# joe5saia/Hmc.jl

Hardware: AMD Instinct MI355X
Metric: Gibbs draws/sec (whole node), 3-state T=1000 x256 windows per GPU (higher is better)
Workload: dtype f64

## Files before the change

hmc.jl_amd/csrc/gibbs_device.hpp:

```cpp
#pragma once
#include <hip/hip_runtime.h>
#include <stdint.h>

#include "../../include/hmcg.h"
#include "round5.hpp"

namespace hmcg {

enum { SITE_SIG2 = 0, SITE_MU = 1, SITE_RHO = 2, SITE_A = 3, SITE_X = 4, SITE_NOISE = 5 };
constexpr int GAMMA_MAX_ATTEMPTS = 64;
constexpr double INVSQRT2PI = 0.3989422804014327;
constexpr double TWO_PI = 6.283185307179586476925286766559;
constexpr double EPS64 = 2.220446049250313e-16;

struct KernelParams {
    const double* Y;
    const int32_t* T;
    const double* yreal;
    int32_t ldY, W, H;
    int32_t sweep_begin;
    int32_t sweep_end;
    int32_t resume;
    int32_t final_launch;
    int32_t horizons[HMCG_MAXH];
// ... 456 lines not shown
__device__ __forceinline__ uint32_t map_const(int v)
{
    uint32_t m = 0;
#pragma unroll
    for (int s = 0; s < K; ++s) m |= (uint32_t)v << (4 * s);
    return m;
}
__device__ __forceinline__ int map_apply(uint32_t m, int s) { return (int)((m >> (4 * s)) & 15u); }

constexpr uint32_t BMAP_IDENTITY = 0x03020100u;
__device__ __forceinline__ uint32_t bmap_const(int v) { return (uint32_t)v * 0x01010101u; }
__device__ __forceinline__ uint32_t bmap_compose(uint32_t a, uint32_t b) { return __builtin_amdgcn_perm(a, a, b); }
__device__ __forceinline__ int bmap_apply(uint32_t m, int s) { return (int)((m >> (8 * s)) & 0xFFu); }
constexpr int DPP_ROW_SHL1 = 0x101, DPP_ROW_SHL2 = 0x102, DPP_ROW_SHL4 = 0x104, DPP_ROW_SHL8 = 0x108, DPP_WAVE_SHL1 = 0x130;

template <int K>
__device__ inline void matmul_small(double (&out)[K][K], const double (&a)[K][K], const double (&b)[K][K])
{
    double t[K][K];
#pragma unroll
    for (int i = 0; i < K; ++i)
#pragma unroll
        for (int j = 0; j < K; ++j) {
            double acc = 0.0;
#pragma unroll
            for (int k = 0; k < K; ++k) acc += a[i][k] * b[k][j];
            t[i][j] = acc;
        }
#pragma unroll
    for (int i = 0; i < K; ++i)
#pragma unroll
        for (int j = 0; j < K; ++j) out[i][j] = t[i][j];
}

template <int K>
__device__ inline double forecast_value(const double (&mu)[K], const double (&A)[K][K], const double (&pe)[K], int h)
{
    double M[K][K], v[K];
#pragma unroll
    for (int i = 0; i < K; ++i) {
        v[i] = mu[i];
#pragma unroll
        for (int j = 0; j < K; ++j) M[i][j] = A[i][j];
    }
    for (unsigned hh = (unsigned)h; hh != 0; hh >>= 1) {
        if (hh & 1u) {
            double nv[K];
#pragma unroll
            for (int i = 0; i < K; ++i) {
                double acc = 0.0;
#pragma unroll
                for (int j = 0; j < K; ++j) acc = fma(M[i][j], v[j], acc);
                nv[i] = acc;
            }
#pragma unroll
            for (int i = 0; i < K; ++i) v[i] = nv[i];
        }
        if (hh > 1u) matmul_small<K>(M, M, M);
    }
    double f = 0.0;
#pragma unroll
    for (int i = 0; i < K; ++i) f = fma(pe[i], v[i], f);
    return f;
}


template <int K>
struct ThetaBuf {
    double mu[K], sig2[K], isd[K], coef[K], rho[K];
    double A[K][K];
    double pi_end[K];
};

template <int K>
struct RngBuf {
    static constexpr int NG = K + K * K;
    double x[NG][2];
    double lu[NG][2];
    double uu[NG][2];
    double z[K];
    double rho[K];
};

template <int K, int L, int NT, bool SIG>
struct SweepShared {
    static constexpr int NW = NT / 64;
    static constexpr int NCNT = K + K * K;
    static constexpr int NF = K * K + (SIG ? K : 0);
    static constexpr int FW = (64 * L < 1024) ? 10 : 16;
    static constexpr int FPK = 32 / FW;
    static constexpr int NPK = (NF + FPK - 1) / FPK;
    unsigned red_pk[NW][NPK];
    double red_s1[SIG ? NW : 1][K];
    double red_s2[SIG ? NW : 1][K];
    int x_end;
    double red_d1[NW][K];
    double red_d2[NW][K];
    double pivot[K];
    ThetaBuf<K> th[2];
    RngBuf<K> rb[2];
    double wtot[NW][K * K];
    double pfirst[NT + 1][K];
    uint32_t wmap[NW];
    double ulast;
    int xfirst[NT + 1];
    double bred[NW];
    int selcnt[2][8][3];
    double ux[NT * L];
    double exptab[EXPTAB_N * EXPTAB_C];
    struct OutConst { double* base; double yr; int packed; int h; };
    OutConst oc[2][64];
    double ftail[2][SIG ? HMCG_MAXTAIL : 1][K];
    double pf_rep[2][K];
    double y_last[2];
};

template <int NW>
__device__ __forceinline__ double block_sum(double v, double* bred, int wave, int lane)
{
    v = wave_sum(v);
    __syncthreads();
    if (lane == 0 && wave < NW) bred[wave] = v;
    __syncthreads();
    double t = 0.0;
#pragma unroll
    for (int w = 0; w < NW; ++w) t += bred[w];
    return t;
}
template <int NW>
__device__ __forceinline__ double block_minmax(double v, double* bred, int wave, int lane, bool is_max)
{
    v = is_max ? wave_max(v) : wave_min(v);
    __syncthreads();
    if (lane == 0 && wave < NW) bred[wave] = v;
    __syncthreads();
    double t = bred[0];
#pragma unroll
    for (int w = 1; w < NW; ++w) t = is_max ? fmax(t, bred[w]) : fmin(t, bred[w]);
    return t;
}

__device__ __forceinline__ unsigned long long order_key(double v)
{
    const long long b = __double_as_longlong(v + 0.0);
    return (unsigned long long)(b ^ ((b >> 63) | (long long)0x8000000000000000ull));
}
__device__ __forceinline__ double key_value(unsigned long long k)
{
    return __longlong_as_double((long long)((k >> 63) ? (k ^ 0x8000000000000000ull) : ~k));
}
template <int NW, int NE, typename ElemFn>
__device__ __forceinline__ unsigned long long block_select(int n, ElemFn elem, int r, int (*cnt)[8][3], int wave, int lane)
{
    unsigned long long prefix = 0ull, mask = 0ull;
    const bool mine = __builtin_amdgcn_readfirstlane(wave) < NW;
    for (int b = 62; b >= 0; b -= 2) {
        const int par = (b >> 1) & 1;
        if (mine) {
            int c0 = 0, c1 = 0, c2 = 0;
            auto one = [&](int i) __attribute__((always_inline)) {
                unsigned long long key;
                const bool live = elem(i, key);
                const bool cand = live && ((key ^ prefix) & mask) == 0ull;
                const unsigned digit = (unsigned)(key >> b) & 3u;
                c0 += __builtin_popcountll(__builtin_amdgcn_ballot_w64(cand && digit == 0u));
                c1 += __builtin_popcountll(__builtin_amdgcn_ballot_w64(cand && digit == 1u));
                c2 += __builtin_popcountll(__builtin_amdgcn_ballot_w64(cand && digit == 2u));
            };
            if constexpr (NE > 0) {
#pragma unroll
                for (int i = 0; i < NE; ++i) one(i);
            } else {
                for (int i = 0; i < n; ++i) one(i);
            }
            if (lane == 0) { cnt[par][wave][0] = c0; cnt[par][wave][1] = c1; cnt[par][wave][2] = c2; }
        }
        __syncthreads();
        int t0 = 0, t1 = 0, t2 = 0;
#pragma unroll
        for (int w = 0; w < NW; ++w) { t0 += cnt[par][w][0]; t1 += cnt[par][w][1]; t2 += cnt[par][w][2]; }
        t0 = __builtin_amdgcn_readfirstlane(t0); t1 = __builtin_amdgcn_readfirstlane(t1); t2 = __builtin_amdgcn_readfirstlane(t2);
        unsigned long long digit = 0ull;
        if (r >= t0) { r -= t0; digit = 1ull;
            if (r >= t1) { r -= t1; digit = 2ull;
                if (r >= t2) { r -= t2; digit = 3ull; } } }
        prefix |= digit << b;
        mask |= 3ull << b;
    }
    return prefix;
}

template <int K>
__device__ __forceinline__ void sort_order(const double (&mu)[K], int (&order)[K])
{
    int pos[K];
#pragma unroll
    for (int i = 0; i < K; ++i) {
        int c = 0;
#pragma unroll
        for (int j = 0; j < K; ++j) c += (mu[j] < mu[i] || (mu[j] == mu[i] && j < i)) ? 1 : 0;
        pos[i] = c;
    }
#pragma unroll
    for (int q = 0; q < K; ++q) {
        int o = 0;
#pragma unroll
        for (int i = 0; i < K; ++i) o += (pos[i] == q) ? i : 0;
        order[q] = o;
    }
}

#ifdef HMCG_STAMPS
#define HMCG_NSTAMP 20
#define HMCG_NSTAMP_ALL (HMCG_NSTAMP + 2)
#define STAMP(i)                                                          \
    do {                                                                  \
        __builtin_amdgcn_sched_barrier(0);                                \
        asm volatile("; HMCG_STAMP_MARK %0" :: "n"(i));                    \
        const unsigned long long t_ = __builtin_amdgcn_s_memtime();       \
        __builtin_amdgcn_s_waitcnt(0xC07F);                               \
        __builtin_amdgcn_sched_barrier(0);                                \
        stamp_acc[i] += t_ - stamp_prev;                                  \
        stamp_prev = t_;                                                  \
    } while (0)
#else
#define STAMP(i)
#endif


template <int K, int L, int NT, bool SIG = false, bool SMOOTH = false, int NH = 0, int OCC = 1>
__global__ __launch_bounds__(NT + 64 * NH) __attribute__((amdgpu_waves_per_eu(OCC)))
void gibbs_sweeps_kernel(const KernelParams p)
{
    static_assert(NH == 0 || (NH == 4 && NT == 256), "helper waves: 256 + 256 threads");
    static_assert(K >= 2 && K <= 4, "small-K kernel: byte-per-entry state maps (v_perm_b32 composition)");
    static_assert(NT % 64 == 0 && NT >= 128, "at least two whole waves (wave 0 draws, the others work in its shadow)");
    constexpr int NW = NT / 64;
    constexpr int KK = K * K;
    constexpr int NG = K + KK;
    static_assert(NG <= 64, "draw roles must fit wave 0");
    using Sh = SweepShared<K, L, NT, SIG>;
    __shared__ Sh sh;

    int w_ = blockIdx.x;
    int t_lo_ = INT32_MIN, t_hi_ = INT32_MAX;
    if (p.order) {
        const int n_live = p.order[0];
        t_lo_ = p.order[1]; t_hi_ = p.order[2];
        if (n_live >= 0) {
            if (w_ >= n_live) __builtin_amdgcn_endpgm();
            w_ = p.order[4 + w_];
        }
    }
    const int w = w_;
    const int tid = threadIdx.x, lane = tid & 63, wave = __builtin_amdgcn_readfirstlane(tid >> 6);
    const int T = p.T[w];
    const int t0 = tid * L;
    const int owner = (T - 1) / L, l_last = (T - 1) % L;
    const bool helper = NH > 0 && __builtin_amdgcn_readfirstlane(wave) >= NW;
    int st = 0;

    if (T < t_lo_ || T > t_hi_) __builtin_amdgcn_endpgm();
    if (T < 2 || T > NT * L || T > p.ldY) {
        if (tid == 0) flag_skipped(p, w, HMCG_ST_BAD_T);
        return;
    }

    exptab_fill(sh.exptab, tid, NT + 64 * NH);
    constexpr int XPAD = K < 4 ? K : 0;
    constexpr bool PADMARK = K < 4;
    double y[L];
    int x[L];
    bool bad = false;
#pragma unroll
    for (int l = 0; l < L; ++l) {
        const bool v = (t0 + l) < T;
        y[l] = v ? p.Y[(size_t)w * p.ldY + t0 + l] : 0.0;
        bad |= v && !isfinite(y[l]);
        x[l] = XPAD;
    }
    if (__syncthreads_or(bad ? 1 : 0)) {
        if (tid == 0) flag_skipped(p, w, HMCG_ST_NONFINITE);
        return;
    }
    int sb = T, se = T;
    double yreal[SIG ? L : 1];
    const double kfac = SIG ? 1.0 / (1.0 + p.kappa) : 1.0;
    if constexpr (SIG) {
        if (p.sig_range) { sb = p.sig_range[2 * w]; se = p.sig_range[2 * w + 1]; }
        bool bad_range = sb < 0 || se > T || (sb < se && se != T);
        if (p.save_range) {
            const int svb = p.save_range[2 * w], sve = p.save_range[2 * w + 1];
            bad_range |= svb < 0 || sve > T || (svb < sve && p.sigvals && sve - svb > p.nsave_ld);
        }
        if (bad_range) {
            if (tid == 0) flag_skipped(p, w, HMCG_ST_BAD_RANGE);
            return;
        }
        if (sb >= se) { sb = T; se = T; }
#pragma unroll
        for (int l = 0; l < L; ++l) yreal[l] = y[l];
    }
    int tail = 0;
    if constexpr (SIG) {
        if (p.end_pos) tail = (T - 1) - p.end_pos[w];
        if (tail < 0 || tail > HMCG_MAXTAIL || tail > T - 1) {
            if (tid == 0) flag_skipped(p, w, HMCG_ST_BAD_T);
            return;
        }
    }
    (void)kfac; (void)yreal; (void)sb; (void)se; (void)tail;

    double part = 0.0;
#pragma unroll
    for (int l = 0; l < L; ++l) part += y[l];
    const double xi = block_sum<NW>(part, sh.bred, wave, lane) / (double)T;

    double pivot[K];
#pragma unroll
    for (int k = 0; k < K; ++k) pivot[k] = xi;

    const int NCK = 3 * K + K * K + 2 * p.H + K;
    if (p.resume) {
#pragma unroll
        for (int l = 0; l < L; ++l) if (t0 + l < T) x[l] = min((int)p.xstate[(size_t)w * p.ldY + t0 + l], K - 1);
        if (p.sumacc) {
#pragma unroll
            for (int k = 0; k < K; ++k) pivot[k] = p.sumacc[(size_t)w * NCK + (NCK - K) + k];
        }
    } else if (p.x_init) {
#pragma unroll
        for (int l = 0; l < L; ++l) if (t0 + l < T) x[l] = min(max(p.x_init[(size_t)w * p.ldY + t0 + l], 0), K - 1);
    } else {
        double lmin = 1.0e308, lmax = -1.0e308;
#pragma unroll
        for (int l = 0; l < L; ++l) if (t0 + l < T) { lmin = fmin(lmin, y[l]); lmax = fmax(lmax, y[l]); }
        const double ymin = block_minmax<NW>(lmin, sh.bred, wave, lane, false);
        const double ymax = block_minmax<NW>(lmax, sh.bred, wave, lane, true);
        unsigned long long key[L];
#pragma unroll
        for (int l = 0; l < L; ++l) key[l] = order_key(y[l]);
        const int rlo = (T - 1) / 2;
        const double med_lo = key_value(block_select<NW, L>(L, [&](int l, unsigned long long& k) __attribute__((always_inline)) { k = key[l]; return t0 + l < T; },
                                                            rlo, sh.selcnt, wave, lane));
        double med_hi = med_lo;
        if (!(T & 1)) {
            double nle = 0.0, above = 1.0e308;
#pragma unroll
            for (int l = 0; l < L; ++l) {
                if (!helper && t0 + l < T) {
                    if (y[l] <= med_lo) nle += 1.0;
                    else above = fmin(above, y[l]);
                }
            }
            const double cle = block_sum<NW>(nle, sh.bred, wave, lane);
            const double nxt = block_minmax<NW>(above, sh.bred, wave, lane, false);
            med_hi = (cle > (double)(rlo + 1)) ? med_lo : nxt;
        }
        {
#pragma clang fp contract(off)
// ... 311 lines not shown
            unsigned v = 0;
#pragma unroll
            for (int q = 0; q < Sh::FPK; ++q) {
                const int e = Sh::FPK * d + q;
                if (e < NF) v |= ((acc[e / FPW] >> (PB * (e % FPW))) & ((1u << PB) - 1u)) << (Sh::FW * q);
            }
            pk[d] = v;
        }
        wave_sum_words_lane63<NPK>(pk);
        double d1[K], d2[K], s1[SIG ? K : 1], s2[SIG ? K : 1];
#pragma unroll
        for (int i = 0; i < K; ++i) { d1[i] = 0.0; d2[i] = 0.0; }
        if constexpr (SIG) {
#pragma unroll
            for (int i = 0; i < K; ++i) { s1[i] = 0.0; s2[i] = 0.0; }
        }
#pragma unroll
        for (int l = 0; l < L; ++l) {
            double pvt = pivot[0];
#pragma unroll
            for (int k = 1; k < K; ++k) pvt = (x[l] == k) ? pivot[k] : pvt;
            const double dl = y[l] - pvt;
            const int t = t0 + l;
            const bool issig = SIG && t >= sb && t < se;
            const int xs = PADMARK ? (issig ? -1 : x[l]) : ((t < T && !issig) ? x[l] : -1);
#pragma unroll
            for (int i = 0; i < K; ++i) {
                const double dm = (xs == i) ? dl : 0.0;
                d1[i] += dm;
                d2[i] = fma(dm, dm, d2[i]);
            }
            if constexpr (SIG) {
                const int xg = issig ? x[l] : -1;
#pragma unroll
                for (int i = 0; i < K; ++i) {
                    const double dm = (xg == i) ? dl : 0.0;
                    s1[i] += dm;
                    s2[i] = fma(dm, dm, s2[i]);
                }
            }
        }
        if constexpr (SIG) {
            static_assert(!SIG || K <= 4, "signal path: transposed reduce carries 2 x 4 slots");
            double v8[8], o0, o1;
#pragma unroll
            for (int i = 0; i < 4; ++i) { v8[i] = i < K ? s1[i < K ? i : 0] : 0.0; v8[4 + i] = i < K ? s2[i < K ? i : 0] : 0.0; }
            wave_sum8_transposed(v8, lane, o0, o1);
            if ((lane & 0x3C) == 12) {
                const int i0 = lane & 2, i1 = i0 + 1;
                double* dst = (lane & 1) ? &sh.red_s2[wave][0] : &sh.red_s1[wave][0];
                if (i0 < K) dst[i0] = o0;
                if (i1 < K) dst[i1] = o1;
            }
        }
        if constexpr (K <= 4) {
            double v8[8], o0, o1;
#pragma unroll
            for (int i = 0; i < 4; ++i) { v8[i] = i < K ? d1[i] : 0.0; v8[4 + i] = i < K ? d2[i] : 0.0; }
            wave_sum8_transposed(v8, lane, o0, o1);
            if ((lane & 0x3C) == 12) {
                const int i0 = lane & 2, i1 = i0 + 1;
                double* dst = (lane & 1) ? &sh.red_d2[wave][0] : &sh.red_d1[wave][0];
                if (i0 < K) dst[i0] = o0;
                if (i1 < K) dst[i1] = o1;
            }
        } else {
#pragma unroll
            for (int i = 0; i < K; ++i) { d1[i] = wave_sum(d1[i]); d2[i] = wave_sum(d2[i]); }
            if (lane == 0) {
#pragma unroll
                for (int i = 0; i < K; ++i) { sh.red_d1[wave][i] = d1[i]; sh.red_d2[wave][i] = d2[i]; }
            }
        }
        if (lane == 63) {
#pragma unroll
            for (int d = 0; d < NPK; ++d) sh.red_pk[wave][d] = pk[d];
        }
        if (tid == 0) {
#pragma unroll
            for (int k = 0; k < K; ++k) sh.pivot[k] = pivot[k];
            sh.x_end = x_end;
        }
    };
    auto regen_y = [&](int smp, bool report) __attribute__((always_inline)) {
        if constexpr (SIG) {
            const double ssig = p.sigma_signal ? p.sigma_signal[w] : 0.0;
            const bool noisy = ssig != 0.0 || p.n_samples > 1;
            int svb = 0, sve = 0;
            if (p.save_range) { svb = p.save_range[2 * w]; sve = p.save_range[2 * w + 1]; }
            Rng gn = rng;
            gn.sweep = (uint32_t)smp;
#pragma unroll
            for (int l = 0; l < L; ++l) {
                const int t = t0 + l;
                if (noisy && t >= sb && t < se) {
                    uint32_t r[4];
                    gn.block(SITE_NOISE, 0, (uint32_t)t, r);
                    y[l] = yreal[l] + box_muller(r) * ssig;
                }
                if (report && p.sigvals && t >= svb && t < sve && t < T && (t - svb) < p.nsave_ld)
                    p.sigvals[((size_t)w * p.n_samples + smp) * p.nsave_ld + (t - svb)] = y[l];
                if (t == T - 1) sh.y_last[smp & 1] = y[l];
            }
        }
    };
    if constexpr (SIG) {
        if (p.sweep_begin % p.per_sample != 0) regen_y(p.sweep_begin / p.per_sample, false);
    }
    if (!helper) publish_stats();

    if (p.sweep_begin < p.sweep_end && shadow_wave == 0) job_prep(p.sweep_begin);

    uint32_t trips = 0;
    if constexpr (NH > 0) {
        const int ntrip = (((T + 1) >> 1) + 127) >> 7;
        constexpr int trip_wave[10] = {1, 2, 3, NW, 1, 2, 3, NW + 3, NW + 2, NW + 1};
        for (int k = 0; k < ntrip && k < 32; ++k) {
            const int wv = k < 10 ? trip_wave[k] : 1 + (k - 10) % 3;
            trips |= (wv == wave) ? (1u << k) : 0u;
        }
        trips = __builtin_amdgcn_readfirstlane(trips);
    }
    auto job_uniform_trips = [&](int sw) __attribute__((always_inline)) {
        const int nblk = (T + 1) >> 1;
        for (uint32_t m = trips; m != 0; m &= m - 1) {
            const int k = __builtin_ctz(m);
            job_uniforms(sw, k << 7, min((k << 7) + 128, nblk));
        }
    };

    double pf[L][K];
    double sm_acc[SMOOTH ? L : 1][K];
    double fm_acc[SMOOTH ? L : 1][K];
    if constexpr (SMOOTH) {
#pragma unroll
        for (int l = 0; l < L; ++l)
#pragma unroll
            for (int q = 0; q < K; ++q)
            {
                sm_acc[l][q] = (p.resume && p.pi_smooth_mean && t0 + l < T) ? p.pi_smooth_mean[((size_t)w * p.ldY + t0 + l) * K + q] : 0.0;
                fm_acc[l][q] = (p.resume && p.pi_filter_mean && t0 + l < T) ? p.pi_filter_mean[((size_t)w * p.ldY + t0 + l) * K + q] : 0.0;
            }
    }
    (void)sm_acc; (void)fm_acc;
#ifdef HMCG_STAMPS
    for (int i = 0; i < HMCG_NSTAMP; ++i) stamp_acc[i] = 0;
    stamp_prev = __builtin_amdgcn_s_memtime();
    const unsigned long long stamp_t0 = stamp_prev, stamp_r0 = __builtin_amdgcn_s_memrealtime();
#endif

    if constexpr (NH > 0) {
        if (helper) {
            for (int sweep = p.sweep_begin; sweep < p.sweep_end; ++sweep) {
                __syncthreads();
                STAMP(0);
                if (wave == PREP_WAVE && sweep + 1 < p.sweep_end) job_prep(sweep + 1);
                STAMP(15);
                job_uniform_trips(sweep);
                STAMP(1);
                __syncthreads();
                STAMP(2);
                if (sweep > p.sweep_begin) job_outputs(sweep - 1);
                STAMP(14);
                __syncthreads();
                __syncthreads();
                __syncthreads();
                STAMP(11);
            }
        }
    }

    for (int sweep = helper ? p.sweep_end : p.sweep_begin; sweep < p.sweep_end; ++sweep) {
        rng.sweep = (uint32_t)sweep;
        const int par = sweep & 1;
        ThetaBuf<K>& th = sh.th[par];
        if constexpr (SIG) {
            const int smp = sweep / p.per_sample;
            if (sweep == smp * p.per_sample) { regen_y(smp, true); publish_stats(); }
        }
        __syncthreads();
        STAMP(0);
        if (wave == 0) {
            const RngBuf<K>& rb = sh.rb[par];
            const int qi = (lane - 4) >> 2, qj = (lane - 4) & 3;
            const bool is_sig = lane < K, is_A = lane >= 4 && qi < K && qj < K;
            const bool is_g = is_sig || is_A;
            const int role = is_sig ? lane : (is_A ? K + qi * K + qj : NG);
            double shape = 1.0, bpar = 1.0, Neff = 0.0, Ssum = 0.0, rnn = 0.0;
            int cT = 0;
            {
                const int e = is_A ? (PADCNT ? qj * K + qi : role - K) : 0;
#pragma unroll
                for (int ww = 0; ww < NW; ++ww) cT += (int)((sh.red_pk[ww][e / Sh::FPK] >> (Sh::FW * (e % Sh::FPK))) & ((1u << Sh::FW) - 1u));
                cT = is_A ? cT : 0;
            }
            int rowsum = 0;
            {
                int qs = cT + __builtin_amdgcn_mov_dpp(cT, 0xB1, 0xF, 0xF, false);
                qs += __builtin_amdgcn_mov_dpp(qs, 0x4E, 0xF, 0xF, false);
#pragma unroll
                for (int i = 0; i < K; ++i) {
                    const int ri = __builtin_amdgcn_readlane(qs, 4 + 4 * i);
                    rowsum = (lane == i) ? ri : rowsum;
                }
            }
            STAMP(16);
            if (is_g) {
                const int c = is_sig ? rowsum + ((sh.x_end == role) ? 1 : 0) : cT;
                if (is_sig) {
                    double d1 = 0.0, d2 = 0.0;
#pragma unroll
                    for (int ww = 0; ww < NW; ++ww) { d1 += sh.red_d1[ww][role]; d2 += sh.red_d2[ww][role]; }
                    const double piv = sh.pivot[role];
                    const double beta = (sweep == 0) ? 1.0 : 2.0;
                    if constexpr (!SIG) {
                        Neff = (double)c;
                        const double rn = c > 0 ? rcp_fast(Neff) : 0.0;
                        const double ybar = c > 0 ? piv + d1 * rn : 0.0;
                        const double S2 = c > 0 ? fmax(d2 - d1 * d1 * rn, 0.0) : 0.0;
                        Ssum = piv * Neff + d1;
                        const double dm = ybar - xi;
                        shape = p.alpha + 0.5 * Neff;
                        rnn = rcp_fast(Neff + p.nu);
                        bpar = beta + 0.5 * S2 + 0.5 * Neff * p.nu * rnn * (dm * dm);
                    } else {
                        int Mi = 0;
                        {
                            const int e = KK + role;
#pragma unroll
                            for (int ww = 0; ww < NW; ++ww) Mi += (int)((sh.red_pk[ww][e / Sh::FPK] >> (Sh::FW * (e % Sh::FPK))) & ((1u << Sh::FW) - 1u));
                        }
                        const int Ni = c - Mi;
                        double g1 = 0.0, g2 = 0.0;
#pragma unroll
                        for (int ww = 0; ww < NW; ++ww) { g1 += sh.red_s1[ww][role]; g2 += sh.red_s2[ww][role]; }
                        const double dNi = (double)Ni, dMi = (double)Mi;
                        const double S = piv * dNi + d1, Sm = piv * dMi + g1;
                        const double S2 = Ni > 0 ? fmax(d2 - d1 * d1 / dNi, 0.0) : 0.0;
                        const double Sm2 = Mi > 0 ? fmax(g2 - g1 * g1 / dMi, 0.0) : 0.0;
                        const double totalbar = (Ni + Mi) > 0 ? (S + Sm) / (dNi + dMi) : 0.0;
                        Neff = dNi + dMi * kfac;
                        Ssum = S + Sm;
                        const double dm = totalbar - xi;
                        shape = p.alpha + 0.5 * dNi + 0.5 * dMi;
                        rnn = rcp_fast(Neff + p.nu);
                        bpar = beta + 0.5 * S2 + (0.5 * kfac) * Sm2 + 0.5 * Neff * p.nu * rnn * (dm * dm);
                    }
                } else {
                    shape = (double)(c + 1);
                }
// ... 455 lines not shown
        STAMP(8);
        int xlast = 0;
        {
            const double ulast = sh.ulast;
            double cp = 0.0;
#pragma unroll
            for (int q = 0; q < K - 1; ++q) {
                double pq = 0.0;
#pragma unroll
                for (int s = 0; s < K; ++s) pq = (order[q] == s) ? th.pi_end[s] : pq;
                cp += pq;
                xlast += (cp <= ulast) ? 1 : 0;
            }
        }
        double pfn_last[K];
#pragma unroll
        for (int s = 0; s < K; ++s) pfn_last[s] = sh.pfirst[(tid + 1 < NT) ? tid + 1 : tid][s];
        uint32_t gmap[L];
        uint32_t G = BMAP_IDENTITY;
#pragma unroll
        for (int l = L - 1; l >= 0; --l) {
            const int t = t0 + l;
            uint32_t m = 0;
            int idx_uni = 0;
            {
                double ucum = 0.0;
#pragma unroll
                for (int r = 0; r < K - 1; ++r) { ucum += 1.0 / K; idx_uni += (ucum <= ux[l]) ? 1 : 0; }
            }
#pragma unroll
            for (int s = 0; s < K; ++s) {
                const double guard = (l + 1 < L) ? pf[(l + 1 < L) ? l + 1 : l][s] : pfn_last[s];
                double tot = 0.0;
                int idx = 0;
                double cum[K];
#pragma unroll
                for (int r = 0; r < K; ++r) { tot = fma(pf[l][r], A[r][s], tot); cum[r] = tot; }
                const double thr = ux[l] * tot;
#pragma unroll
                for (int r = 0; r < K - 1; ++r) idx += (cum[r] <= thr) ? 1 : 0;
                idx = (guard > EPS64) ? idx : idx_uni;
                m |= (uint32_t)idx << (8 * s);
            }
            if constexpr (K < 4) m |= BMAP_IDENTITY & (0xFFFFFFFFu << (8 * K));
            m = (t == T - 1) ? bmap_const(xlast) : (t > T - 1 ? (PADMARK ? bmap_const(XPAD) : BMAP_IDENTITY) : m);
            gmap[l] = m;
            G = bmap_compose(m, G);
        }
        STAMP(9);
        uint32_t Hm = G;
        Hm = bmap_compose(Hm, (uint32_t)dpp_i32<DPP_ROW_SHL1, 0xF>((int)BMAP_IDENTITY, (int)Hm));
        Hm = bmap_compose(Hm, (uint32_t)dpp_i32<DPP_ROW_SHL2, 0xF>((int)BMAP_IDENTITY, (int)Hm));
        Hm = bmap_compose(Hm, (uint32_t)dpp_i32<DPP_ROW_SHL4, 0xF>((int)BMAP_IDENTITY, (int)Hm));
        Hm = bmap_compose(Hm, (uint32_t)dpp_i32<DPP_ROW_SHL8, 0xF>((int)BMAP_IDENTITY, (int)Hm));
        {
            const uint32_t R1 = (uint32_t)__builtin_amdgcn_readlane((int)Hm, 16);
            const uint32_t R2 = (uint32_t)__builtin_amdgcn_readlane((int)Hm, 32);
            const uint32_t R3 = (uint32_t)__builtin_amdgcn_readlane((int)Hm, 48);
            const uint32_t S1 = bmap_compose(R2, R3), S0 = bmap_compose(R1, S1);
            const int row = lane >> 4;
            const uint32_t after = row == 0 ? S0 : (row == 1 ? S1 : (row == 2 ? R3 : BMAP_IDENTITY));
            Hm = bmap_compose(Hm, after);
        }
        if (lane == 0) sh.wmap[wave] = Hm;
        STAMP(10);
        __syncthreads();
        STAMP(11);
        uint32_t Rw = BMAP_IDENTITY;
#pragma unroll
        for (int ww = NW - 1; ww >= 1; --ww) if (ww > wave_u) Rw = bmap_compose(sh.wmap[ww], Rw);
        const uint32_t Hx = (uint32_t)dpp_i32<DPP_WAVE_SHL1, 0xF>((int)BMAP_IDENTITY, (int)Hm);
        const uint32_t Sfx = bmap_compose(Hx, Rw);
        int sin = bmap_apply(Sfx, XPAD);
        xnext = sin;
        x_end = xlast;
#pragma unroll
        for (int l = L - 1; l >= 0; --l) {
            sin = bmap_apply(gmap[l], sin);
            x[l] = sin;
        }
#pragma unroll
        for (int k = 0; k < K; ++k) pivot[k] = mu[k];
        STAMP(12);
        publish_stats();
        STAMP(13);
    }
#ifdef HMCG_STAMPS
    if (lane == 0 && p.dbg) {
        unsigned long long* o = p.dbg + ((size_t)w * (NW + NH) + wave) * HMCG_NSTAMP_ALL;
        for (int i = 0; i < HMCG_NSTAMP; ++i) o[i] = stamp_acc[i];
        o[HMCG_NSTAMP] = __builtin_amdgcn_s_memtime() - stamp_t0;
        o[HMCG_NSTAMP + 1] = __builtin_amdgcn_s_memrealtime() - stamp_r0;
    }
#endif

    __syncthreads();
    if (p.sweep_end > p.sweep_begin) job_outputs(p.sweep_end - 1);
    if (p.xstate) {
#pragma unroll
        for (int l = 0; l < L; ++l) if (t0 + l < T) p.xstate[(size_t)w * p.ldY + t0 + l] = (uint8_t)x[l];
    }
    if (p.x_final) {
#pragma unroll
        for (int l = 0; l < L; ++l) if (t0 + l < T) p.x_final[(size_t)w * p.ldY + t0 + l] = x[l];
    }
    if (p.pif_final && p.sweep_end > p.sweep_begin) {
#pragma unroll
        for (int l = 0; l < L; ++l)
            if (t0 + l < T)
#pragma unroll
                for (int s = 0; s < K; ++s) p.pif_final[((size_t)w * p.ldY + t0 + l) * K + s] = pf[l][s];
    }
    if constexpr (SMOOTH) {
        if (p.pi_filter_mean) {
            const double sc = (p.final_launch && p.nd > 0) ? 1.0 / (double)p.nd : 1.0;
#pragma unroll
            for (int l = 0; l < L; ++l)
                if (t0 + l < T)
#pragma unroll
                    for (int q = 0; q < K; ++q) p.pi_filter_mean[((size_t)w * p.ldY + t0 + l) * K + q] = fm_acc[l][q] * sc;
        }
        if (p.pi_smooth_mean) {
            const double sc = (p.final_launch && p.nd > 0) ? 1.0 / (double)p.nd : 1.0;
#pragma unroll
            for (int l = 0; l < L; ++l)
                if (t0 + l < T)
#pragma unroll
                    for (int q = 0; q < K; ++q) p.pi_smooth_mean[((size_t)w * p.ldY + t0 + l) * K + q] = sm_acc[l][q] * sc;
        }
    }
    {
        const int orole = role_of(lane);
        if (orole >= 0) {
            if (p.sumacc) p.sumacc[(size_t)w * NCK + orole] = sum_acc;
            if (p.summary && p.final_launch)
                p.summary[(size_t)w * NS + orole] = p.nd > 0 ? sum_acc / (double)p.nd : __builtin_nan("");
            if constexpr (SIG) {
                if (p.sample_summary) {
                    const int smp = p.sweep_end / p.per_sample, kb = p.sweep_end - smp * p.per_sample - p.burnin_s;
                    if (kb > 0 && kb < p.nrun_s && smp < p.n_samples) p.sample_summary[((size_t)w * p.n_samples + smp) * NS + orole] = smp_acc;
                }
            }
        }
    }
    if (p.sumacc) {
#pragma unroll
        for (int k = 0; k < K; ++k) if (tid == k) p.sumacc[(size_t)w * NCK + (NCK - K) + k] = pivot[k];
    }
    if (st) atomicOr(&p.status[w], st);
}

}
```

hmc.jl_amd/csrc/hmcg.hip:

```cpp
#include <hip/hip_runtime.h>

#include <algorithm>
#include <chrono>
#include <cstdarg>
#include <cstdlib>
#include <cstdio>
#include <cstring>
#include <functional>
#include <mutex>
#include <string>
#include <thread>
#include <vector>

#include "gibbs_device.hpp"
#include "host_util.hpp"
#include "moments.hpp"
#include "plan.hpp"

namespace {

thread_local char g_err[512] = "";

void set_err(const char* fmt, ...)
{
// ... 249 lines not shown
{
    const size_t stride = (size_t)W + ORD_HDR;
    int32_t* meta = ord + (size_t)MAXBUCKET * stride;
    const int w = (int)(blockIdx.x * blockDim.x + threadIdx.x);
    if (w < W) {
        auto bucket_of = [&](int t) { int k = 0; for (int b = 0; b < r.nb; ++b) if (t >= r.lo[b] && t <= r.hi[b]) k = b; return k; };
        const int mine = bucket_of(T[w]);
        int32_t* list = ord + (size_t)mine * stride;
        const int pos = atomicAdd(&list[0], 1);
        list[ORD_HDR + pos] = w;
        if (w > 0 && bucket_of(T[w - 1]) != mine) atomicAdd(&meta[0], 1);
    }
    __threadfence();
    __syncthreads();
    if (threadIdx.x == 0 && atomicAdd(&meta[1], 1) == (int)gridDim.x - 1) {
        __threadfence();
        int runs = 0;
        for (int b = 0; b < r.nb; ++b) runs += atomicAdd(&ord[(size_t)b * stride], 0) > 0 ? 1 : 0;
        const bool sorted = atomicAdd(&meta[0], 0) == runs - 1 || !r.compact;
        for (int b = 0; b < r.nb; ++b) {
            int32_t* list = ord + (size_t)b * stride;
            if (sorted) list[0] = -1;
            list[1] = r.lo[b]; list[2] = r.hi[b];
        }
    }
}
size_t bucket_list_bytes(int W) { return sizeof(int32_t) * ((size_t)MAXBUCKET * ((size_t)W + ORD_HDR) + 2); }
int build_bucket_lists(const Plan& pl, const int32_t* dT, int W, int32_t* ord, hipStream_t stream)
{
    BucketRanges r{};
    r.nb = pl.nb;
    r.compact = diag_env("HMCG_NO_BUCKET_LISTS") ? 0 : 1;
    for (int b = 0; b < pl.nb; ++b) { r.lo[b] = pl.b[b].t_lo; r.hi[b] = pl.b[b].t_hi; }
    HIP_TRY(hipMemsetAsync(ord, 0, bucket_list_bytes(W), stream));
    hipLaunchKernelGGL(bucket_lists_kernel, dim3((unsigned)((W + 255) / 256)), dim3(256), 0, stream, dT, W, r, ord);
    HIP_TRY(hipGetLastError());
    return 0;
}

int launch_kernel(DeviceCtx& c, const Plan& pl, const hmcg::KernelParams& p, hipStream_t stream, const int32_t* ord)
{
    if (pl.nb > 1) {
        HIP_TRY(hipEventRecord(c.ev_fork, stream));
        for (int b = 0; b < pl.nb; ++b) {
            hipStream_t bs = b == 0 ? stream : c.bstream[b - 1];
            if (b > 0) HIP_TRY(hipStreamWaitEvent(bs, c.ev_fork, 0));
            hmcg::KernelParams q = p;
            q.order = ord + (size_t)b * ((size_t)p.W + ORD_HDR);
            const Variant* v = pl.b[b].v;
            hipLaunchKernelGGL(v->fn, dim3((unsigned)p.W), dim3((unsigned)(v->NT + 64 * v->NH)), 0, bs, q);
            HIP_TRY(hipGetLastError());
            if (b > 0) HIP_TRY(hipEventRecord(c.ev_join[b - 1], bs));
        }
        for (int b = 1; b < pl.nb; ++b) HIP_TRY(hipStreamWaitEvent(stream, c.ev_join[b - 1], 0));
        return 0;
    }
    if (pl.v) hipLaunchKernelGGL(pl.v->fn, dim3((unsigned)p.W), dim3((unsigned)(pl.v->NT + 64 * pl.v->NH)), 0, stream, p);
    else hipLaunchKernelGGL(pl.bv->fn, dim3((unsigned)p.W), dim3((unsigned)pl.bv->NT), pl.dyn, stream, p, pl.bigL);
    HIP_TRY(hipGetLastError());
    return 0;
}

void fill_timing(hmcg_timing* t, const Plan& pl, const DeviceCtx& c, double kernel_ms, int launches, double call_ms, int windows)
{
    if (!t) return;
    t->kernel_ms = kernel_ms;
    t->launches = launches;
    t->threads_per_window = pl.NT();
    t->steps_per_thread = pl.L();
    t->helper_waves = pl.NH();
    t->device = c.device;
    t->call_ms = call_ms;
    t->windows = windows;
    t->occupancy = pl.v ? pl.v->occ : 0;
    t->buckets = pl.nb > 1 ? pl.nb : 1;
    t->streaming = pl.stream ? 1 : 0;
    t->lds_bytes = (int32_t)(static_lds_bytes(pl.fptr(), 0) + pl.dyn);
}

#ifdef HMCG_STAMPS
int print_stamps(const hmcg::KernelParams& p, const Plan& pl, unsigned long long* ddbg, size_t ndbg, hipStream_t stream)
{
    static const char* names[HMCG_NSTAMP] = {"Ba wait", "param draws | shadow jobs", "Bb wait", "theta+ux+pdfs", "local product",
        "wave scan", "Bc wait", "prefix+replay+last", "Bd wait", "maps+compose", "map scan", "Be wait", "apply", "publish stats", "  (shadow: outputs)", "  (shadow: prep)", "  (param: counts+row sums)", "  (param: shapes)", "  (param: gamma)", "unused"};
    const int nwv = pl.NT() / 64 + pl.NH();
    std::vector<unsigned long long> h(ndbg);
    HIP_TRY(hipStreamSynchronize(stream));
    static int launches_seen = 0;
    static const int print_after = diag_env("HMCG_STAMPS_AFTER") ? atoi(diag_env("HMCG_STAMPS_AFTER")) : 0;
    if (launches_seen++ < print_after) return 0;
    HIP_TRY(hipMemcpy(h.data(), ddbg, ndbg * sizeof(unsigned long long), hipMemcpyDeviceToHost));
    const int nsw = p.sweep_end - p.sweep_begin;
    {
        std::vector<double> clk;
        double ticks = 0;
        for (int w = 0; w < p.W; ++w)
            for (int wv = 0; wv < nwv; ++wv) {
                const unsigned long long* o = &h[((size_t)w * nwv + wv) * HMCG_NSTAMP_ALL];
                if (o[HMCG_NSTAMP + 1]) { clk.push_back(100.0 * (double)o[HMCG_NSTAMP] / (double)o[HMCG_NSTAMP + 1]); ticks += (double)o[HMCG_NSTAMP]; }
            }
        std::sort(clk.begin(), clk.end());
        if (!clk.empty())
            fprintf(stderr, "[clock] launch %d: in-kernel clock MHz min %.0f median %.0f max %.0f (s_memtime / s_memrealtime x 100 MHz); "
                            "%.0f ticks per sweep (mean over waves)\n", launches_seen - 1, clk.front(), clk[clk.size() / 2], clk.back(),
                    ticks / (double)clk.size() / (nsw > 0 ? nsw : 1));
    }
    fprintf(stderr, "[stamps] K=%d L=%d NT=%d W=%d sweeps=%d: mean cycles per sweep by wave (s_memtime ticks)\n",
            pl.v ? pl.v->K : pl.bv->K, pl.L(), pl.NT(), p.W, nsw);
    fprintf(stderr, "%-24s", "phase");
    for (int wv = 0; wv < nwv; ++wv) fprintf(stderr, "   wave%-2d", wv);
    fprintf(stderr, "\n");
    std::vector<double> tot(nwv, 0.0);
    for (int i = 0; i < HMCG_NSTAMP; ++i) {
        fprintf(stderr, "%-24s", names[i]);
        for (int wv = 0; wv < nwv; ++wv) {
            double acc = 0;
            for (int w = 0; w < p.W; ++w) acc += (double)h[((size_t)w * nwv + wv) * HMCG_NSTAMP_ALL + i];
            acc /= (double)p.W * (nsw > 0 ? nsw : 1);
            tot[wv] += acc;
            fprintf(stderr, " %8.0f", acc);
        }
        fprintf(stderr, "\n");
    }
    fprintf(stderr, "%-24s", "total");
    for (int wv = 0; wv < nwv; ++wv) fprintf(stderr, " %8.0f", tot[wv]);
    fprintf(stderr, "\n");
    return 0;
}
#endif


int grow_shared(DeviceCtx& c, Arena& a, size_t bytes)
{
    if (a.cap >= bytes) return 0;
    HIP_TRY(hipEventSynchronize(c.ev_scr));
    if (a.ensure(bytes)) { set_err("workspace allocation failed (%zu B device)", bytes); return HMCG_E_NOMEM; }
    return 0;
}

int launch_device(DeviceCtx& c, const hmcg_config* cfg, const double* dY, const int32_t* dT, const double* dyreal, double* dmu,
                  double* dsig2, double* dA, double* dpi_end, double* dfcast, double* dsummary, int32_t* dstatus,
                  const hmcg_extras* ex, hipStream_t stream, hmcg_timing* timing)
{
    if (!dY || !dT || !dstatus) { set_err("Y, T and status are required"); return HMCG_E_BADARG; }
    Plan pl;
    int rc = plan_call(cfg, ex, cfg->W, c.cu_count, cfg->min_T, nullptr, &pl);
    if (rc) return rc;
    if (pl.needs_pif() && !(ex && ex->pif_final)) {
        set_err("pi_smooth_mean / pi_filter_mean for K >= 5 or windows beyond the register-resident kernels need extras.pif_final "
                "([W][ldY][K]: the running sweep's filtered probabilities pass through it)");
        return HMCG_E_BADARG;
    }
    if (ex && ex->corr && (!dmu || !dsig2 || !dA || !dpi_end || !dfcast)) {
        set_err("extras.corr on the device entry needs all five per-draw outputs");
        return HMCG_E_BADARG;
    }
    const bool resume = (cfg->flags & HMCG_FLAG_RESUME) != 0;
    hmcg::KernelParams p = base_params(cfg, cfg->W, dY, dT, dyreal, dstatus, ex, pl);
    p.sweep_begin = pl.sched.sweep_begin; p.sweep_end = pl.sched.sweep_end; p.final_launch = pl.sched.final_launch;
    p.resume = resume ? 1 : 0;
    p.mu = dmu; p.sig2 = dsig2; p.A = dA; p.pi_end = dpi_end; p.fcast = dfcast; p.summary = dsummary;
    p.nd_ld = p.nd; p.draw_off = 0;

    if (!resume) HIP_TRY(hipMemsetAsync(dstatus, 0, sizeof(int32_t) * (size_t)cfg->W, stream));
    const bool use_lists = pl.nb > 1;
    const bool uses_scratch = pl.bv != nullptr || (ex && ex->corr) || use_lists;
    if (uses_scratch) HIP_TRY(hipStreamWaitEvent(stream, c.ev_scr, 0));
// ... 454 lines not shown
```

Measured before the change: 54.11 million.

## Offload per-state residual sums to helper waves via shared state bytes

When helper waves are present (non-SIG, non-smooth), the main waves now pack their sampled state sequence into shared memory as bytes. After an extra barrier, helper waves load those states along with their own copy of y and compute the per-state first and second moment sums, while main waves compute only the transition counts. This splits the end-of-sweep statistics work across more waves so the critical path gets shorter. In exchange it adds an extra __syncthreads per sweep and uses more LDS for the state bytes.

```diff
diff --git a/hmc.jl_amd/csrc/gibbs_device.hpp b/hmc.jl_amd/csrc/gibbs_device.hpp
--- a/hmc.jl_amd/csrc/gibbs_device.hpp
+++ b/hmc.jl_amd/csrc/gibbs_device.hpp
@@ -562,8 +562,11 @@
     double rho[K];
 };
 
-template <int K, int L, int NT, bool SIG>
-struct SweepShared {
+template <int NXS> struct StateBytes { uint32_t xs[NXS]; };
+template <> struct StateBytes<0> {};
+
+template <int K, int L, int NT, bool SIG, int NXS = 0>
+struct SweepShared : StateBytes<NXS> {
     static constexpr int NW = NT / 64;
     static constexpr int NCNT = K + K * K;
     static constexpr int NF = K * K + (SIG ? K : 0);
@@ -719,7 +722,9 @@
     constexpr int KK = K * K;
     constexpr int NG = K + KK;
     static_assert(NG <= 64, "draw roles must fit wave 0");
-    using Sh = SweepShared<K, L, NT, SIG>;
+    constexpr bool HSTAT = NH > 0 && !SIG && !SMOOTH && !(K == 2 && L >= 3);
+    constexpr int XSW = (L + 3) / 4;
+    using Sh = SweepShared<K, L, NT, SIG, HSTAT ? NT * XSW : 0>;
     __shared__ Sh sh;
 
     int w_ = blockIdx.x;
@@ -738,6 +743,7 @@
     const int t0 = tid * L;
     const int owner = (T - 1) / L, l_last = (T - 1) % L;
     const bool helper = NH > 0 && __builtin_amdgcn_readfirstlane(wave) >= NW;
+    const int ts = (HSTAT && helper) ? t0 - NT * L : t0;
     int st = 0;
 
     if (T < t_lo_ || T > t_hi_) __builtin_amdgcn_endpgm();
@@ -754,8 +760,8 @@
     bool bad = false;
 #pragma unroll
     for (int l = 0; l < L; ++l) {
-        const bool v = (t0 + l) < T;
-        y[l] = v ? p.Y[(size_t)w * p.ldY + t0 + l] : 0.0;
+        const bool v = (ts + l) < T;
+        y[l] = v ? p.Y[(size_t)w * p.ldY + ts + l] : 0.0;
         bad |= v && !isfinite(y[l]);
         x[l] = XPAD;
     }
@@ -1233,6 +1239,102 @@
             sh.x_end = x_end;
         }
     };
+    auto stats_counts = [&]() __attribute__((always_inline)) {
+        unsigned acc[NWORD];
+#pragma unroll
+        for (int wd = 0; wd < NWORD; ++wd) acc[wd] = 0;
+#pragma unroll
+        for (int l = 0; l < L; ++l) {
+            const int xn = (l + 1 < L) ? x[(l + 1 < L) ? l + 1 : l] : xnext;
+            const int code = PADCNT ? x[l] + K * xn : x[l] * K + xn;
+            const bool pv = (t0 + l + 1) < T;
+            if constexpr (PADCNT) {
+                acc[0] += 1u << (PB * min(code, KK));
+            } else if constexpr (NWORD == 1) {
+                acc[0] += pv ? (1u << (PB * code)) : 0u;
+            } else {
+#pragma unroll
+                for (int wd = 0; wd < NWORD; ++wd) {
+                    const int rel = code - wd * FPW;
+                    acc[wd] += (pv && rel >= 0 && rel < FPW) ? (1u << (PB * rel)) : 0u;
+                }
+            }
+        }
+        unsigned pk[NPK];
+#pragma unroll
+        for (int d = 0; d < NPK; ++d) {
+            unsigned v = 0;
+#pragma unroll
+            for (int q = 0; q < Sh::FPK; ++q) {
+                const int e = Sh::FPK * d + q;
+                if (e < NF) v |= ((acc[e / FPW] >> (PB * (e % FPW))) & ((1u << PB) - 1u)) << (Sh::FW * q);
+            }
+            pk[d] = v;
+        }
+        wave_sum_words_lane63<NPK>(pk);
+        if (lane == 63) {
+#pragma unroll
+            for (int d = 0; d < NPK; ++d) sh.red_pk[wave][d] = pk[d];
+        }
+        if (tid == 0) {
+#pragma unroll
+            for (int k = 0; k < K; ++k) sh.pivot[k] = pivot[k];
+            sh.x_end = x_end;
+        }
+    };
+    auto stats_sums = [&]() __attribute__((always_inline)) {
+        double d1[K], d2[K];
+#pragma unroll
+        for (int i = 0; i < K; ++i) { d1[i] = 0.0; d2[i] = 0.0; }
+#pragma unroll
+        for (int l = 0; l < L; ++l) {
+            double pvt = pivot[0];
+#pragma unroll
+            for (int k = 1; k < K; ++k) pvt = (x[l] == k) ? pivot[k] : pvt;
+            const double dl = y[l] - pvt;
+            const int xs = PADMARK ? x[l] : ((ts + l < T) ? x[l] : -1);
+#pragma unroll
+            for (int i = 0; i < K; ++i) {
+                const double dm = (xs == i) ? dl : 0.0;
+                d1[i] += dm;
+                d2[i] = fma(dm, dm, d2[i]);
+            }
+        }
+        double v8[8], o0, o1;
+#pragma unroll
+        for (int i = 0; i < 4; ++i) { v8[i] = i < K ? d1[i < K ? i : 0] : 0.0; v8[4 + i] = i < K ? d2[i < K ? i : 0] : 0.0; }
+        wave_sum8_transposed(v8, lane, o0, o1);
+        if ((lane & 0x3C) == 12) {
+            const int i0 = lane & 2, i1 = i0 + 1;
+            const int wrow = helper ? wave - NW : wave;
+            double* dst = (lane & 1) ? &sh.red_d2[wrow][0] : &sh.red_d1[wrow][0];
+            if (i0 < K) dst[i0] = o0;
+            if (i1 < K) dst[i1] = o1;
+        }
+    };
+    auto store_states = [&]() __attribute__((always_inline)) {
+        if constexpr (HSTAT) {
+#pragma unroll
+            for (int q = 0; q < XSW; ++q) {
+                unsigned v = 0;
+#pragma unroll
+                for (int b = 0; b < 4; ++b)
+                    if (4 * q + b < L) v |= (unsigned)x[(4 * q + b < L) ? 4 * q + b : 0] << (8 * b);
+                sh.xs[tid * XSW + q] = v;
+            }
+        }
+    };
+    auto load_states = [&]() __attribute__((always_inline)) {
+        if constexpr (HSTAT) {
+#pragma unroll
+            for (int q = 0; q < XSW; ++q) {
+                const unsigned v = sh.xs[(tid - NT) * XSW + q];
+#pragma unroll
+                for (int b = 0; b < 4; ++b)
+                    if (4 * q + b < L) x[(4 * q + b < L) ? 4 * q + b : 0] = (int)((v >> (8 * b)) & 0xFFu);
+            }
+        }
+    };
     auto regen_y = [&](int smp, bool report) __attribute__((always_inline)) {
         if constexpr (SIG) {
             const double ssig = p.sigma_signal ? p.sigma_signal[w] : 0.0;
@@ -1258,7 +1360,18 @@
     if constexpr (SIG) {
         if (p.sweep_begin % p.per_sample != 0) regen_y(p.sweep_begin / p.per_sample, false);
     }
-    if (!helper) publish_stats();
+    if constexpr (HSTAT) {
+        if (!helper) store_states();
+        __syncthreads();
+        if (helper) {
+            load_states();
+            stats_sums();
+        } else {
+            stats_counts();
+        }
+    } else {
+        if (!helper) publish_stats();
+    }
 
     if (p.sweep_begin < p.sweep_end && shadow_wave == 0) job_prep(p.sweep_begin);
 
@@ -1317,6 +1430,15 @@
                 __syncthreads();
                 __syncthreads();
                 STAMP(11);
+                if constexpr (HSTAT) {
+                    __syncthreads();
+                    STAMP(19);
+                    load_states();
+#pragma unroll
+                    for (int k = 0; k < K; ++k) pivot[k] = sh.th[sweep & 1].mu[k];
+                    stats_sums();
+                    STAMP(13);
+                }
             }
         }
     }
@@ -1938,7 +2060,14 @@
 #pragma unroll
         for (int k = 0; k < K; ++k) pivot[k] = mu[k];
         STAMP(12);
-        publish_stats();
+        if constexpr (HSTAT) {
+            store_states();
+            __syncthreads();
+            STAMP(19);
+            stats_counts();
+        } else {
+            publish_stats();
+        }
         STAMP(13);
     }
 #ifdef HMCG_STAMPS
diff --git a/hmc.jl_amd/csrc/hmcg.hip b/hmc.jl_amd/csrc/hmcg.hip
--- a/hmc.jl_amd/csrc/hmcg.hip
+++ b/hmc.jl_amd/csrc/hmcg.hip
@@ -355,7 +355,7 @@
 int print_stamps(const hmcg::KernelParams& p, const Plan& pl, unsigned long long* ddbg, size_t ndbg, hipStream_t stream)
 {
     static const char* names[HMCG_NSTAMP] = {"Ba wait", "param draws | shadow jobs", "Bb wait", "theta+ux+pdfs", "local product",
-        "wave scan", "Bc wait", "prefix+replay+last", "Bd wait", "maps+compose", "map scan", "Be wait", "apply", "publish stats", "  (shadow: outputs)", "  (shadow: prep)", "  (param: counts+row sums)", "  (param: shapes)", "  (param: gamma)", "unused"};
+        "wave scan", "Bc wait", "prefix+replay+last", "Bd wait", "maps+compose", "map scan", "Be wait", "apply", "publish stats", "  (shadow: outputs)", "  (shadow: prep)", "  (param: counts+row sums)", "  (param: shapes)", "  (param: gamma)", "Bs wait"};
     const int nwv = pl.NT() / 64 + pl.NH();
     std::vector<unsigned long long> h(ndbg);
     HIP_TRY(hipStreamSynchronize(stream));
```

Result: no change. 54.47 million, median of 6 (+0.7%).
